# clawrim/gcn10

Hardware: AMD Instinct MI355X
Metric: CN Gpixels/sec (higher is better)
Workload: dtype u8

## Files before the change

gcn10_amd/csrc/gcn10_deflate_fused.hip:

```cpp
#include <hip/hip_runtime.h>

#include <cstdint>
#include <cstring>

#include "gcn10_deflate_internal.hpp"
#include "gcn10_gpu.h"
#include "gcn10_gpu_internal.hpp"

using gcn10::as_stream;
using gcn10::fail;
using gcn10::u32x4;
using gcn10::use_device;
using namespace gcn10_deflate;

namespace {

constexpr int kGroup = 6;

struct FusedJob {
    const uint8_t *esa;
    const uint8_t *hx;
    const int32_t *cj;
    const uint8_t *class_of;
    uint16_t *tok;
// ... 1338 lines not shown
    if (!ctx->d_hx || ctx->hx_W == 0 || (uint32_t)W != ctx->hx_W)
        return fail(GCN10_E_STATE, "gcn10_gpu_deflate_fused_strip: call gcn10_gpu_prepare_tile for W=%d first", W);
    if (W <= 0 || rows < 0 || cond_mask == 0 || (cond_mask & ~3u) || table_mask == 0 ||
        (table_mask >> ctx->n_tables))
        return fail(GCN10_E_INVAL, "gcn10_gpu_deflate_fused_strip: bad shape or masks");
    if (rows == 0)
        return GCN10_OK;
    if (!esa || !cj || !arena_dev || !table_dev || !cursor_dev)
        return fail(GCN10_E_INVAL, "gcn10_gpu_deflate_fused_strip: null pointer");
    if ((reinterpret_cast<uintptr_t>(arena_dev) & 15u) != 0)
        return fail(GCN10_E_INVAL, "gcn10_gpu_deflate_fused_strip: arena must be 16-byte aligned");

    FusedJob job;
    memset(&job, 0, sizeof job);
    job.esa = esa;
    job.hx = ctx->d_hx;
    job.cj = cj;
    job.class_of = ctx->d_class_of;
    job.hx_stride = ctx->hx_stride;
    job.hx_rows = ctx->hx_rows;
    job.seg_align = (uint32_t)ctx->arena_segment_align;
    for (int r = 0; r < GCN10_N_RASTERS; r++)
        if ((cond_mask >> (r / 9)) & 1u && (table_mask >> (r % 9)) & 1u)
            job.sel[job.n_sel++] = (uint8_t)r;
    job.t.arena = arena_dev;
    job.t.table = table_dev;
    job.t.cursor = cursor_dev;
    job.t.W = (uint32_t)W;
    job.t.rows = (uint32_t)rows;
    job.t.across = ((uint32_t)W + kTile - 1) / kTile;
    job.t.down = ((uint32_t)rows + kTile - 1) / kTile;
// ... 62 lines not shown
```

gcn10_amd/csrc/gcn10_gpu.hip:

```cpp

#include <hip/hip_runtime.h>
#include <unistd.h>
#include <hip/hip_ext.h>

#include <cstdarg>
#include <cstdint>
#include <cstdio>
#include <cstdlib>
#include <cstring>
#include <new>

#include "gcn10_gpu.h"
#include "gcn10_gpu_internal.hpp"

using gcn10::as_stream;
using gcn10::fail;
using gcn10::u32x4;
using gcn10::use_device;

namespace {

constexpr int kThreads = 256;
constexpr int kPxPerLane = 16;
constexpr int kChunk = kThreads * kPxPerLane;
// ... 11 lines not shown
    const uint8_t *hx;
    const int32_t *cj;
    const uint8_t *lut;
    uint8_t *out[GCN10_N_RASTERS];
    uint32_t W;
    uint32_t rows;
    uint32_t npix;
    uint32_t nvec16;
    uint32_t hx_stride;
    uint32_t hx_rows;
    uint32_t nchunks;
    uint32_t table_mask;
    uint32_t single_k;
    uint32_t xcd_slabs;
    const uint32_t *hx4;
    const uint32_t *hx4_complex;
    uint32_t hx4_stride;
    uint32_t hx4_gen;
};

__host__ __device__ inline uint8_t soil_code(uint8_t h)
{
    uint8_t d, u;
    if (h >= 11 && h <= 14) {
        d = 4;
        u = (uint8_t)(h - 10);
    }
    else {
        d = u = (h < 5) ? h : (uint8_t)kInvalidPlane;
    }
    return (uint8_t)(d | (u << 4));
}

// ... 80 lines not shown
        uint32_t lo = xcd * per;
        uint32_t hi = lo + per < nchunks ? lo + per : nchunks;
        step = nb / 8u;
        end = hi;
        return lo + (b >> 3);
    }
    step = nb;
    end = nchunks;
    return b;
}

enum { kLut16 = 0, kLut1 = 1 };
constexpr uint32_t kWavePx = 64u * kPxPerLane;
constexpr uint32_t kMinVectorW = kWavePx + 16u;

template <int ILP>
struct Trip {
    u32x4 e16[ILP], c16[ILP];
    uint32_t i0[ILP];
};

template <int ILP, bool NT, bool HX4>
__device__ __forceinline__ void issue_trip(const StripParams &p, uint32_t trip, uint32_t lane_off,
                                           uint32_t wave_off, Trip<ILP> &tr)
{
    uint32_t xb[ILP], r0[ILP], r1[ILP], wb[ILP];
#pragma unroll
    for (int u = 0; u < ILP; u++) {
        wb[u] = __builtin_amdgcn_readfirstlane((trip * ILP + u) * (uint32_t)kChunk + wave_off);
        const uint32_t wbc = wb[u] < p.npix ? wb[u] : 0u;
        const uint32_t y = wbc / p.W;
        xb[u] = wbc - y * p.W;
        r0[u] = (uint32_t)scalar_load_i32(p.cj, y);
        r1[u] = (uint32_t)scalar_load_i32(p.cj, y + 1u < p.rows ? y + 1u : y);
    }
#pragma unroll
    for (int u = 0; u < ILP; u++) {
        tr.i0[u] = wb[u] + lane_off;
        const uint8_t *pe = p.esa + (tr.i0[u] < p.nvec16 ? tr.i0[u] : 0u);
        tr.e16[u] = NT ? load16_aligned_nt(pe) : load16_aligned(pe);
    }
#pragma unroll
    for (int u = 0; u < ILP; u++) {
        uint32_t xl = xb[u] + lane_off;
        const bool wrap = xl >= p.W;
        xl = wrap ? xl - p.W : xl;
        const uint32_t row = clamp_row(p, (int32_t)(wrap ? r1[u] : r0[u]));
        if (HX4) {
            tr.c16[u] = u32x4{ p.hx4[(size_t)row * p.hx4_stride + (xl >> 4)], 0u, 0u, 0u };
            continue;
        }
        const uint8_t *pa = p.hx + (size_t)row * p.hx_stride + xl;
        u32x4 a = load16_any(pa);
        if (p.W & 15u) {
            const uint32_t n = p.W - xl;
            const bool strad = !wrap && n < (uint32_t)kPxPerLane;
            if (__builtin_amdgcn_ballot_w64(strad) != 0ull) {
                const uint8_t *pb = strad ? p.hx + (size_t)clamp_row(p, (int32_t)r1[u]) * p.hx_stride - n : pa;
                const u32x4 b = load16_any(pb);
                const uint32_t nn = strad ? n : (uint32_t)kPxPerLane;
#pragma unroll
                for (int j = 0; j < 4; j++) {
                    const int32_t m = (int32_t)nn - 4 * j;
                    const uint32_t mask = m >= 4 ? 0xffffffffu : (m <= 0 ? 0u : (1u << (8 * m)) - 1u);
// ... 7 lines not shown

__device__ __forceinline__ u32x4 expand_soil_word(uint32_t w)
{
    const uint32_t a = (w & 0xffu) * 0x01010101u, b = ((w >> 8) & 0xffu) * 0x01010101u;
    const int32_t split = (int32_t)((w >> 16) & 0xffu);
    u32x4 cd;
#pragma unroll
    for (int j = 0; j < 4; j++) {
        const int32_t m = split - 4 * j;
        const uint32_t mask = m >= 4 ? 0xffffffffu : (m <= 0 ? 0u : (1u << (8 * m)) - 1u);
        cd[j] = (a & mask) | (b & ~mask);
    }
    return cd;
}

template <int KIND, int COND_MASK, int ILP, bool NT, bool HX4>
__device__ __forceinline__ void finish_trip(const StripParams &p, const uint8_t *lut, uint32_t tmask,
                                            const Trip<ILP> &tr)
{
#pragma unroll
    for (int u = 0; u < ILP; u++) {
        const bool live = tr.i0[u] < p.nvec16;
        const u32x4 c16 = HX4 ? expand_soil_word(tr.c16[u][0]) : tr.c16[u];
#pragma unroll
        for (int c = 0; c < 2; c++) {
            if (!(COND_MASK & (1 << c)))
                continue;
            if (KIND == kLut16) {
                uint32_t acc[9][4];
#pragma unroll
                for (int j = 0; j < 4; j++) {
                    const uint32_t e = tr.e16[u][j];
                    const uint32_t cd = c16[j];
                    u32x4 r4[4];
#pragma unroll
                    for (int q = 0; q < 4; q++) {
                        const uint32_t lc16 = q == 0 ? (e << 4) & 0xff0u : (e >> (8 * q - 4)) & 0xff0u;
                        const uint32_t s = (cd >> (8 * q + 4 * c)) & 0xfu;
// ... 27 lines not shown
                    for (int q = 0; q < 4; q++) {
                        const uint32_t lc = (e >> (8 * q)) & 0xffu;
                        const uint32_t s = (cd >> (8 * q + 4 * c)) & 0xfu;
                        const uint32_t b = lut[s * (uint32_t)kPlane1 + lc];
                        w |= b << (8 * q);
                    }
                    v[j] = w;
                }
                if (live)
                    store16<NT>(p.out[c * 9 + p.single_k] + tr.i0[u], v);
            }
        }
    }
}

template <int KIND, int COND_MASK, int ILP, bool NT, bool PF, bool HX4>
__device__ __forceinline__ void strip_loop(const StripParams &p, const uint8_t *lut, uint32_t tmask,
                                           uint32_t lane_off, uint32_t wave_off)
{
    uint32_t step, end;
    uint32_t trip = first_chunk(p.nchunks, step, end, p.xcd_slabs != 0);
    if (!PF) {
        for (; trip < end; trip += step) {
            Trip<ILP> tr;
            issue_trip<ILP, NT, HX4>(p, trip, lane_off, wave_off, tr);
            finish_trip<KIND, COND_MASK, ILP, NT, HX4>(p, lut, tmask, tr);
        }
    }
    else if (trip < end) {
        Trip<ILP> ta, tb;
        issue_trip<ILP, NT, HX4>(p, trip, lane_off, wave_off, ta);
        for (;;) {
            trip += step;
            if (trip >= end) {
                finish_trip<KIND, COND_MASK, ILP, NT, HX4>(p, lut, tmask, ta);
                break;
            }
            issue_trip<ILP, NT, HX4>(p, trip, lane_off, wave_off, tb);
            finish_trip<KIND, COND_MASK, ILP, NT, HX4>(p, lut, tmask, ta);
            trip += step;
            if (trip >= end) {
                finish_trip<KIND, COND_MASK, ILP, NT, HX4>(p, lut, tmask, tb);
                break;
            }
            issue_trip<ILP, NT, HX4>(p, trip, lane_off, wave_off, ta);
            finish_trip<KIND, COND_MASK, ILP, NT, HX4>(p, lut, tmask, tb);
        }
    }
}

template <int KIND, int COND_MASK, bool ALL_TABLES, int ILP, bool NT, bool PF>
__global__ __launch_bounds__(kThreads) void cn_strip_kernel(const StripParams p)
{
    constexpr int kLutBytes = KIND == kLut16 ? kLut16Bytes : kLut1Bytes;
    __shared__ __attribute__((aligned(16))) uint8_t lut[kLutBytes];

    if (KIND == kLut16) {
        const u32x4 *src = reinterpret_cast<const u32x4 *>(p.lut);
        u32x4 *dst = reinterpret_cast<u32x4 *>(lut);
        for (int i = threadIdx.x; i < kLutBytes / 16; i += kThreads)
            dst[i] = src[i];
    }
    else {
        const uint32_t *src = reinterpret_cast<const uint32_t *>(p.lut);
        uint32_t *dst = reinterpret_cast<uint32_t *>(lut);
        for (int i = threadIdx.x; i < kLutBytes / 4; i += kThreads)
            dst[i] = src[i];
    }
    __syncthreads();

    const uint32_t lane_off = (threadIdx.x & 63u) * kPxPerLane;
    const uint32_t wave_off = __builtin_amdgcn_readfirstlane(threadIdx.x >> 6) * kWavePx;
    const uint32_t tmask = ALL_TABLES ? 0x1ffu : p.table_mask;

    if (p.hx4 && (uint32_t)scalar_load_i32(reinterpret_cast<const int32_t *>(p.hx4_complex), 0u) != p.hx4_gen)
        strip_loop<KIND, COND_MASK, ILP, NT, PF, true>(p, lut, tmask, lane_off, wave_off);
    else
        strip_loop<KIND, COND_MASK, ILP, NT, PF, false>(p, lut, tmask, lane_off, wave_off);

    if (blockIdx.x == 0 && threadIdx.x < p.npix - p.nvec16) {
        const uint32_t i = p.nvec16 + threadIdx.x;
        const uint32_t y = i / p.W;
        const uint32_t x = i - y * p.W;
        const uint32_t lc = p.esa[i];
        const uint32_t cd = p.hx[(size_t)soil_row(p, y) * p.hx_stride + x];
#pragma unroll
        for (int c = 0; c < 2; c++) {
            if (!(COND_MASK & (1 << c)))
                continue;
            const uint32_t s = (cd >> (4 * c)) & 0xfu;
            if (KIND == kLut16) {
                const uint8_t *row = lut + s * (uint32_t)kPlane16 + lc * 16u;
                for (int k = 0; k < 9; k++)
// ... 40 lines not shown
        const uint32_t x = i - y * p.W;
        const uint32_t lc = p.esa[i];
        const uint32_t cd = p.hx[(size_t)soil_row(p, y) * p.hx_stride + x];
        for (int c = 0; c < 2; c++) {
            if (!(cond_mask & (1u << c)))
                continue;
            const uint32_t s = (cd >> (4 * c)) & 0xfu;
            const uint8_t *row = lut + s * (uint32_t)kPlane16 + lc * 16u;
            for (int k = 0; k < 9; k++)
                if (p.table_mask & (1u << k))
                    p.out[c * 9 + k][i] = row[k];
        }
    }
}

constexpr uint32_t kExpandRows = 4;

template <bool VEC>
__global__ __launch_bounds__(kThreads) void expand_x_codes(const uint8_t *coarse,
                                                           uint32_t hsx, uint32_t hsy,
                                                           const int32_t *ci, uint32_t W,
                                                           uint8_t *hx, uint32_t hx_stride,
                                                           uint32_t *hx4, uint32_t *complex, uint32_t gen)
{
    const uint32_t x = (blockIdx.x * blockDim.x + threadIdx.x) * 16u;
    const uint32_t r0 = blockIdx.y * kExpandRows;
    if (x >= hx_stride || r0 >= hsy)
        return;
    const uint8_t pad = (uint8_t)(kInvalidPlane | (kInvalidPlane << 4));
    uint32_t cx[16];
    if (VEC && x + 16u <= W) {
        const u32x4 *civ = reinterpret_cast<const u32x4 *>(ci + x);
#pragma unroll
        for (int j = 0; j < 4; j++) {
            const u32x4 c4 = civ[j];
#pragma unroll
            for (int q = 0; q < 4; q++)
                cx[4 * j + q] = c4[q] < hsx ? c4[q] : hsx - 1u;
        }
    }
    else {
#pragma unroll
        for (int q = 0; q < 16; q++) {
            const uint32_t xx = x + q;
            const uint32_t c = xx < W ? (uint32_t)ci[xx] : 0u;
            cx[q] = xx < W ? (c < hsx ? c : hsx - 1u) : 0xffffffffu;
        }
    }
    const uint32_t c_lo = cx[0], c_hi = cx[15];
    const uint32_t r1 = r0 + kExpandRows < hsy ? r0 + kExpandRows : hsy;
    uint32_t split = 0;
    bool compact = true, in_set = true;
#pragma unroll
    for (int q = 0; q < 16; q++) {
        const bool lo = cx[q] == c_lo;
        in_set = in_set && (lo || cx[q] == c_hi);
        compact = compact && (lo ? split == (uint32_t)q : cx[q] == c_hi);
        split += lo && split == (uint32_t)q ? 1u : 0u;
    }
    const bool two = c_lo != 0xffffffffu && c_hi != 0xffffffffu && in_set;
    if (hx4 && x < W && !compact && *reinterpret_cast<volatile uint32_t *>(complex) != gen)
        *reinterpret_cast<volatile uint32_t *>(complex) = gen;
    for (uint32_t r = r0; r < r1; r++) {
        const uint8_t *row = coarse + (size_t)r * hsx;
        u32x4 o;
        if (two) {
            const uint32_t code_lo = soil_code(row[c_lo]), code_hi = soil_code(row[c_hi]);
#pragma unroll
            for (int j = 0; j < 4; j++) {
                uint32_t w = 0;
#pragma unroll
                for (int q = 0; q < 4; q++)
                    w |= (cx[4 * j + q] == c_lo ? code_lo : code_hi) << (8 * q);
                o[j] = w;
            }
        }
        else {
#pragma unroll
            for (int j = 0; j < 4; j++) {
                uint32_t w = 0;
#pragma unroll
                for (int q = 0; q < 4; q++) {
                    const uint32_t c = cx[4 * j + q];
                    const uint8_t code = c == 0xffffffffu ? pad : soil_code(row[c]);
                    w |= (uint32_t)code << (8 * q);
                }
                o[j] = w;
            }
        }
        __builtin_nontemporal_store(o, reinterpret_cast<u32x4 *>(hx + (size_t)r * hx_stride + x));
        if (hx4)
            __builtin_nontemporal_store(compact ? (o[0] & 0xffu) | ((o[3] >> 24) << 8) | (split << 16) : 0x00ff0000u,
                                        hx4 + (size_t)r * (hx_stride / 16u) + x / 16u);
    }
}

__global__ __launch_bounds__(kThreads) void resample_rows(const uint8_t *coarse,
                                                          uint32_t hsx,
                                                          const int32_t *ci,
                                                          const int32_t *cj, uint32_t W,
                                                          uint32_t rows, uint8_t *out)
{
    const size_t npix = (size_t)W * rows;
    const size_t stride = (size_t)gridDim.x * blockDim.x;
    for (size_t i = (size_t)blockIdx.x * blockDim.x + threadIdx.x; i < npix; i += stride) {
        const uint32_t y = (uint32_t)(i / W);
        const uint32_t x = (uint32_t)(i - (size_t)y * W);
        out[i] = coarse[(size_t)(uint32_t)cj[y] * hsx + (uint32_t)ci[x]];
// ... 183 lines not shown
{
    return s ? reinterpret_cast<hipStream_t>(s) : ctx->main_stream;
}

int grow_workspace(void **ws, size_t *cap, size_t need)
{
    if (need <= *cap)
        return GCN10_OK;
    HIP_TRY(hipDeviceSynchronize());
    if (*ws)
        HIP_TRY(hipFree(*ws));
    *ws = nullptr;
    *cap = 0;
    HIP_TRY(hipMalloc(ws, need));
    *cap = need;
    return GCN10_OK;
}

}

namespace {

uint32_t stream_grid(const gcn10_gpu_ctx *ctx, uint64_t nchunks, int blocks_per_cu = 0)
{
    uint64_t cap = (uint64_t)ctx->n_cus * (blocks_per_cu > 0 ? blocks_per_cu : ctx->grid_blocks_per_cu);
    cap -= cap % 8u;
    if (cap < 8)
        cap = 8;
    uint64_t g = nchunks < cap ? nchunks : cap;
    return (uint32_t)(g ? g : 1);
// ... 38 lines not shown
    HIP_TRY(hipGetDeviceProperties(&prop, device));
    if (strncmp(prop.gcnArchName, "gfx950", 6) != 0)
        return fail(GCN10_E_NODEVICE, "device %d is %s; this library carries gfx950 code only",
                    device, prop.gcnArchName);

    gcn10_gpu_ctx *ctx = new (std::nothrow) gcn10_gpu_ctx();
    if (!ctx)
        return fail(GCN10_E_NOMEM, "context allocation failed");
    ctx->device = device;
    ctx->n_cus = prop.multiProcessorCount;
    hipError_t e2 = hipStreamCreateWithFlags(&ctx->main_stream, hipStreamNonBlocking);
    if (e2 == hipSuccess)
        e2 = hipMalloc(reinterpret_cast<void **>(&ctx->d_lut16), kLut16Bytes);
    if (e2 == hipSuccess)
        e2 = hipMalloc(reinterpret_cast<void **>(&ctx->d_lut1), GCN10_N_TABLES * kLut1Bytes);
    if (e2 != hipSuccess) {
        int rc = fail(GCN10_E_HIP, "context setup: %s", hipGetErrorString(e2));
        gcn10_gpu_destroy(ctx);
        return rc;
    }
    *out = ctx;
    return GCN10_OK;
}

void gcn10_gpu_destroy(gcn10_gpu_ctx *ctx)
{
    if (!ctx)
        return;
    (void)hipSetDevice(ctx->device);
    if (ctx->main_stream) {
        (void)hipStreamSynchronize(ctx->main_stream);
        (void)hipStreamDestroy(ctx->main_stream);
    }
    if (ctx->d_lut16)
        (void)hipFree(ctx->d_lut16);
    if (ctx->d_lut1)
        (void)hipFree(ctx->d_lut1);
    if (ctx->d_hx_alloc)
        (void)hipFree(ctx->d_hx_alloc);
    if (ctx->deflate_ws)
        (void)hipFree(ctx->deflate_ws);
    if (ctx->inflate_ws)
        (void)hipFree(ctx->inflate_ws);
    if (ctx->lzw_ws)
        (void)hipFree(ctx->lzw_ws);
    if (ctx->d_class_of)
        (void)hipFree(ctx->d_class_of);
    delete ctx;
}

int gcn10_gpu_device_info(gcn10_gpu_ctx *ctx, char *name, size_t cap, size_t *hbm_bytes)
{
    int rc = use_device(ctx);
    if (rc)
// ... 369 lines not shown
    return GCN10_OK;
}


int gcn10_gpu_prepare_tile(gcn10_gpu_ctx *ctx, const uint8_t *coarse, int hsx, int hsy,
                           const int32_t *ci, int W, gcn10_stream_t stream)
{
    int rc = use_device(ctx);
    if (rc)
        return rc;
    if (hsx <= 0 || hsy <= 0 || W <= 0)
        return fail(GCN10_E_INVAL, "gcn10_gpu_prepare_tile: bad shape W=%d soil=%dx%d", W, hsx, hsy);
    if (!coarse || !ci)
        return fail(GCN10_E_INVAL, "gcn10_gpu_prepare_tile: null pointer");
    const uint32_t stride = (((uint32_t)W + 15u) & ~15u) + 16u;
    const size_t need = (size_t)stride * (size_t)hsy;
    if (need > ctx->hx_capacity) {
        HIP_TRY(hipDeviceSynchronize());
        if (ctx->d_hx_alloc)
            HIP_TRY(hipFree(ctx->d_hx_alloc));
        ctx->d_hx_alloc = ctx->d_hx = nullptr;
        ctx->d_hx4 = ctx->d_hx4_complex = nullptr;
        ctx->hx4_ready = false;
        ctx->hx_capacity = 0;
        const size_t need16 = (need + 15) & ~(size_t)15;
        HIP_TRY(hipMalloc(reinterpret_cast<void **>(&ctx->d_hx_alloc), 16 + need16 + need16 / 4 + 16));
        ctx->d_hx = ctx->d_hx_alloc + 16;
        ctx->d_hx4 = reinterpret_cast<uint32_t *>(ctx->d_hx + need16);
        ctx->d_hx4_complex = reinterpret_cast<uint32_t *>(ctx->d_hx + need16 + need16 / 4);
        HIP_TRY(hipMemsetAsync(ctx->d_hx4_complex, 0, 4, as_stream(ctx, stream)));
        ctx->hx4_gen = 0;
        ctx->hx_capacity = need;
    }
    uint32_t *hx4 = ctx->compact_soil ? ctx->d_hx4 : nullptr;
    ctx->hx4_ready = hx4 != nullptr;
    if (hx4 && ++ctx->hx4_gen == 0u)
        ctx->hx4_gen = 1u;
    ctx->hx_stride = stride;
    ctx->hx_W = (uint32_t)W;
    ctx->hx_rows = (uint32_t)hsy;
    dim3 grid((stride / 16 + kThreads - 1) / kThreads, ((uint32_t)hsy + kExpandRows - 1) / kExpandRows);
    if (aligned16(ci))
        hipLaunchKernelGGL(expand_x_codes<true>, grid, dim3(kThreads), 0, as_stream(ctx, stream),
                           coarse, (uint32_t)hsx, (uint32_t)hsy, ci, (uint32_t)W, ctx->d_hx, stride, hx4,
                           ctx->d_hx4_complex, ctx->hx4_gen);
    else
        hipLaunchKernelGGL(expand_x_codes<false>, grid, dim3(kThreads), 0, as_stream(ctx, stream),
                           coarse, (uint32_t)hsx, (uint32_t)hsy, ci, (uint32_t)W, ctx->d_hx, stride, hx4,
                           ctx->d_hx4_complex, ctx->hx4_gen);
    HIP_TRY(hipGetLastError());
    return GCN10_OK;
}

int gcn10_gpu_cn_strip(gcn10_gpu_ctx *ctx, const uint8_t *esa, int W, int rows,
                       const int32_t *cj, unsigned cond_mask, unsigned table_mask,
                       uint8_t *const out[GCN10_N_RASTERS], gcn10_stream_t stream)
{
    int rc = use_device(ctx);
    if (rc)
        return rc;
    if (ctx->n_tables == 0)
        return fail(GCN10_E_STATE, "gcn10_gpu_cn_strip: call gcn10_gpu_set_tables first");
    if (!ctx->d_hx || ctx->hx_W == 0)
        return fail(GCN10_E_STATE, "gcn10_gpu_cn_strip: call gcn10_gpu_prepare_tile first");
    if (W <= 0 || rows < 0 || (uint32_t)W != ctx->hx_W)
// ... 14 lines not shown
    StripParams p;
    memset(&p, 0, sizeof p);
    bool all_aligned = aligned16(esa);
    for (int c = 0; c < 2; c++) {
        for (int k = 0; k < 9; k++) {
            const int r = c * 9 + k;
            if ((cond_mask & (1u << c)) && (table_mask & (1u << k))) {
                if (!out[r])
                    return fail(GCN10_E_INVAL, "gcn10_gpu_cn_strip: out[%d] is null but selected", r);
                p.out[r] = out[r];
                all_aligned = all_aligned && aligned16(out[r]);
            }
        }
    }
    p.esa = esa;
    p.hx = ctx->d_hx;
    p.cj = cj;
    p.W = (uint32_t)W;
    p.rows = (uint32_t)rows;
    p.npix = (uint32_t)((uint64_t)W * (uint64_t)rows);
    p.hx_stride = ctx->hx_stride;
    p.hx_rows = ctx->hx_rows;
    p.nchunks = (p.npix + kChunk - 1) / kChunk;
    p.table_mask = table_mask;
    hipStream_t s = as_stream(ctx, stream);

    p.xcd_slabs = (uint32_t)ctx->xcd_slabs;
    p.nvec16 = p.npix & ~15u;
    if (ctx->hx4_ready && ctx->compact_soil && (p.W & 15u) == 0u) {
        p.hx4 = ctx->d_hx4;
        p.hx4_complex = ctx->d_hx4_complex;
        p.hx4_stride = ctx->hx_stride / 16u;
        p.hx4_gen = ctx->hx4_gen;
    }
    if (p.npix < 16u || p.W < kMinVectorW)
        all_aligned = false;
    if (!all_aligned) {
        p.lut = ctx->d_lut16;
        const uint32_t g = stream_grid(ctx, ((uint64_t)p.npix + kThreads - 1) / kThreads);
        if (ctx->time_start && ctx->time_stop) {
            void *args[] = { &p, &cond_mask };
            HIP_TRY(hipExtLaunchKernel(reinterpret_cast<const void *>(cn_strip_bytes), dim3(g), dim3(kThreads), args, 0,
                                       s, ctx->time_start, ctx->time_stop, 0));
            ctx->time_start = ctx->time_stop = nullptr;
        }
        else {
            hipLaunchKernelGGL(cn_strip_bytes, dim3(g), dim3(kThreads), 0, s, p, cond_mask);
        }
        ctx->last_kernel = "cn_strip_bytes";
    }
    else {
// ... 225 lines not shown
        *best_ms = best;
    if (report && report_cap)
        snprintf(report, report_cap,
                 "{\"positions\": %d, \"step_bytes\": %zu, \"shapes\": %zu, \"best_ms\": %.4f, \"worst_ms\": %.4f, "
                 "\"best_offset_bytes\": %zu, \"xcd_slabs\": %d, \"grid_blocks_per_cu\": %d, \"ilp1\": %d, \"prefetch\": %d}",
                 n_pos, step, sizeof shapes / sizeof shapes[0], best, worst, best_pos, best_shape.xcd, best_shape.bpc,
                 best_shape.ilp, best_shape.pf);
    return GCN10_OK;
}

int gcn10_gpu_soil_words_state(gcn10_gpu_ctx *ctx, gcn10_stream_t stream)
{
    int rc = use_device(ctx);
    if (rc)
        return rc;
    if (!ctx->hx4_ready || !ctx->d_hx4_complex)
        return 0;
    uint32_t flag = 0;
    hipStream_t s = as_stream(ctx, stream);
    HIP_TRY(hipMemcpyAsync(&flag, ctx->d_hx4_complex, 4, hipMemcpyDeviceToHost, s));
    HIP_TRY(hipStreamSynchronize(s));
    return flag == ctx->hx4_gen ? 2 : 1;
}

const char *gcn10_gpu_last_kernel_name(gcn10_gpu_ctx *ctx)
{
    return ctx ? ctx->last_kernel : "";
}

}
```

gcn10_amd/csrc/gcn10_gpu_internal.hpp:

```cpp
#ifndef GCN10_GPU_INTERNAL_HPP
#define GCN10_GPU_INTERNAL_HPP

#include <hip/hip_runtime.h>

#include <cstdint>

#include "gcn10_gpu.h"

namespace gcn10 {

int fail(int code, const char *fmt, ...) __attribute__((format(printf, 2, 3)));

#define HIP_TRY(expr)                                                                   \
    do {                                                                                \
        hipError_t e_ = (expr);                                                         \
        if (e_ != hipSuccess)                                                           \
            return gcn10::fail(e_ == hipErrorOutOfMemory ? GCN10_E_NOMEM : GCN10_E_HIP, \
                               "%s: %s", #expr, hipGetErrorString(e_));                 \
    } while (0)

int use_device(gcn10_gpu_ctx *ctx);
hipStream_t as_stream(gcn10_gpu_ctx *ctx, gcn10_stream_t s);
int grow_workspace(void **ws, size_t *cap, size_t need);

typedef uint32_t u32x4 __attribute__((ext_vector_type(4)));

__device__ __forceinline__ bool inflate_window_ok(uint32_t out_len, uint32_t chunk_w, uint32_t src_x, uint32_t src_y,
                                                  uint32_t copy_w, uint32_t copy_h, uint32_t slot_bytes)
{
    if (copy_w == 0 || copy_h == 0)
        return true;
    if (chunk_w == 0 || out_len > slot_bytes || src_x > chunk_w || copy_w > chunk_w - src_x)
        return false;
    const unsigned long long last = (unsigned long long)(src_y + copy_h - 1u) * chunk_w + src_x + copy_w;
    return (unsigned long long)src_y + copy_h <= 0xffffffffull && last <= out_len;
}

void launch_lzw_decode(const uint8_t *comp_dev, const gcn10_inflate_tile *tiles_dev, uint32_t n_tiles,
// ... 4 lines not shown
constexpr int kLut16Plane = 256 * 16 + 16;
constexpr int kLut16Bytes = 6 * kLut16Plane;

}

struct gcn10_gpu_ctx {
    int device = -1;
    int n_cus = 0;
    hipStream_t main_stream = nullptr;
    uint8_t *d_lut16 = nullptr;
    uint8_t *d_lut1 = nullptr;
    int n_tables = 0;
    uint8_t *d_hx = nullptr;
    uint8_t *d_hx_alloc = nullptr;
    uint32_t *d_hx4 = nullptr;
    uint32_t *d_hx4_complex = nullptr;
    uint32_t hx4_gen = 0;
    bool hx4_ready = false;
    int compact_soil = 1;
    size_t hx_capacity = 0;
    uint32_t hx_stride = 0;
    uint32_t hx_W = 0;
    uint32_t hx_rows = 0;
    const char *last_kernel = "";
    char kernel_name[96] = "";
    int grid_blocks_per_cu = 16;
    int ilp16 = 0;
    int ilp1 = 2;
    int nontemporal = 1;
    int xcd_slabs = 1;
    int prefetch = 1;
    struct SingleShape {
        bool set = false;
        int xcd_slabs = 1, grid_blocks_per_cu = 8, ilp = 2, prefetch = 1;
// ... 22 lines not shown
```

gcn10_amd/csrc/gcn10_overview.hip:

```cpp
#include <hip/hip_runtime.h>

#include <cstdint>

#include "gcn10_gpu_internal.hpp"

using namespace gcn10;

namespace {

constexpr int kThreads = 256;
constexpr int kPlanes = 6;
constexpr int kPlane16 = 256 * 16 + 16;
constexpr int kLut16Bytes = kPlanes * kPlane16;
constexpr int kMaxLevels = 8;
constexpr int kL1Tile = 128;
constexpr uint32_t kL1Rows = 4;

__device__ __forceinline__ uint8_t avg_of(uint32_t s, uint32_t n)
{
    return n == 0 ? (uint8_t)GCN10_NODATA : (uint8_t)((2u * s + n) / (2u * n));
}

struct NearestParams {
    const uint8_t *src;
// ... 173 lines not shown
        return rc;
    if (ctx->n_tables == 0)
        return fail(GCN10_E_STATE, "gcn10_gpu_overview_average: call gcn10_gpu_set_tables first");
    if (!ctx->d_hx || (int)ctx->hx_W != W)
        return fail(GCN10_E_STATE, "gcn10_gpu_overview_average: prepare the block's tile (W=%d) first", W);
    if (!esa || !cj || !levels || W <= 0 || H <= 0 || n_levels < 1 || n_levels > kMaxLevels || y0 < 0 ||
        rows <= 0 || y0 % 256 != 0 || y0 + rows > H || (rows % 256 != 0 && y0 + rows != H))
        return fail(GCN10_E_INVAL, "gcn10_gpu_overview_average: bad strip y0=%d rows=%d of %dx%d, %d levels "
                    "(strips start and end on multiples of 256 rows, 1..8 levels)", y0, rows, W, H, n_levels);
    if (cond_mask == 0 || (cond_mask & ~3u) || table_mask == 0 || (table_mask >> ctx->n_tables) != 0)
        return fail(GCN10_E_INVAL, "gcn10_gpu_overview_average: bad masks cond=%#x table=%#x", cond_mask, table_mask);
    AvgParams p = {};
    p.esa = esa;
    p.cj = cj;
    p.lut16 = ctx->d_lut16;
    p.hx = ctx->d_hx;
    p.hx_stride = ctx->hx_stride;
    p.hx_rows = ctx->hx_rows;
    p.W = (uint32_t)W;
    p.H = (uint32_t)H;
    p.cond_mask = cond_mask;
    p.table_mask = table_mask;
    p.n_levels = (uint32_t)n_levels;
    int q = 0;
    for (int r = 0; r < GCN10_N_RASTERS; r++) {
        if (!((cond_mask >> (r / 9)) & 1u) || !((table_mask >> (r % 9)) & 1u))
            continue;
        for (int k = 0; k < n_levels; k++) {
            p.out[r][k] = levels[q * n_levels + k];
            if (!p.out[r][k])
                return fail(GCN10_E_INVAL, "gcn10_gpu_overview_average: level %d of raster %d is NULL", k + 1, r);
// ... 21 lines not shown
```

gcn10_amd/csrc/gcn10_stats.hip:

```cpp
#include <hip/hip_runtime.h>

#include <cstdint>

#include "gcn10_gpu_internal.hpp"
#include "gcn10_pair_hist.hpp"

using namespace gcn10;
using namespace gcn10::pair_hist;

namespace {

constexpr uint32_t kChunk = kThreads * kPxPerLane;
constexpr uint32_t kRowsPerItem = 4;
constexpr int kGridPerCu = 4;

struct HistParams {
    const uint8_t *esa;
    const uint8_t *hx;
    const int32_t *cj;
    unsigned long long *hist;
    uint32_t W, rows, hx_stride, hx_rows, per_row;
};

__global__ __launch_bounds__(kThreads) void pair_histogram_kernel(const HistParams p)
// ... 63 lines not shown

int gcn10_gpu_pair_histogram(gcn10_gpu_ctx *ctx, const uint8_t *esa, int W, int rows, const int32_t *cj,
                             unsigned long long *hist_dev, gcn10_stream_t stream)
{
    int rc = use_device(ctx);
    if (rc)
        return rc;
    if (!ctx->d_hx || (int)ctx->hx_W != W)
        return fail(GCN10_E_STATE, "gcn10_gpu_pair_histogram: prepare the block's tile (W=%d) first", W);
    if (!esa || !cj || !hist_dev || W <= 0 || rows < 0)
        return fail(GCN10_E_INVAL, "gcn10_gpu_pair_histogram: bad arguments W=%d rows=%d", W, rows);
    if (rows == 0)
        return GCN10_OK;
    HistParams p = {};
    p.esa = esa;
    p.hx = ctx->d_hx;
    p.cj = cj;
    p.hist = hist_dev;
    p.W = (uint32_t)W;
    p.rows = (uint32_t)rows;
    p.hx_stride = ctx->hx_stride;
    p.hx_rows = ctx->hx_rows;
    p.per_row = ((uint32_t)W + kChunk - 1u) / kChunk;
    const uint64_t items = (uint64_t)((p.rows + kRowsPerItem - 1u) / kRowsPerItem) * p.per_row;
    const uint64_t cap = (uint64_t)(ctx->n_cus > 0 ? ctx->n_cus : 256) * kGridPerCu;
    const uint32_t grid = (uint32_t)(items < cap ? items : cap);
    hipLaunchKernelGGL(pair_histogram_kernel, dim3(grid), dim3(kThreads), 0, as_stream(ctx, stream), p);
    HIP_TRY(hipGetLastError());
    return GCN10_OK;
}

// ... 2 lines not shown
```

gcn10_amd/csrc/gcn10_verify.hip:

```cpp
#include <hip/hip_runtime.h>

#include <cstdint>
#include <cstring>

#include "gcn10_gpu_internal.hpp"

using namespace gcn10;

namespace {

constexpr int kThreads = 256;
constexpr uint32_t kPxPerLane = 16;
constexpr int kGridPerCu = 4;

struct VerifyParams {
    const uint8_t *esa;
    const uint8_t *hx;
    const int32_t *cj;
    const uint8_t *lut;
    const uint8_t *want[GCN10_N_RASTERS];
    const uint8_t *got[GCN10_N_RASTERS];
    gcn10_verify_count *counts;
    uint64_t want_stride, got_stride;
    uint32_t W, rows, y0;
// ... 318 lines not shown
        return GCN10_OK;
    if (!esa || !cj || !got || !counts_dev)
        return fail(GCN10_E_INVAL, "gcn10_gpu_verify_strip: null pointer");
    for (int c = 0; c < GCN10_N_CONDS; c++) {
        for (int k = 0; k < GCN10_N_TABLES; k++) {
            const int r = c * GCN10_N_TABLES + k;
            if (!(cond_mask & (1u << c)) || !(table_mask & (1u << k)))
                continue;
            if (!got[r])
                return fail(GCN10_E_INVAL, "gcn10_gpu_verify_strip: got[%d] is null but selected", r);
            p.got[r] = got[r];
            p.sel |= 1u << r;
        }
    }
    p.esa = esa;
    p.hx = ctx->d_hx;
    p.cj = cj;
    p.lut = ctx->d_lut16;
    p.counts = counts_dev;
    p.hx_stride = ctx->hx_stride;
    p.hx_rows = ctx->hx_rows;
    hipStream_t s = as_stream(ctx, stream);
    if (p.sel == (1u << GCN10_N_RASTERS) - 1u)
        hipLaunchKernelGGL(verify_strip_kernel<true>, dim3(grid_for(ctx, p)), dim3(kThreads), 0, s, p);
    else
        hipLaunchKernelGGL(verify_strip_kernel<false>, dim3(grid_for(ctx, p)), dim3(kThreads), 0, s, p);
    HIP_TRY(hipGetLastError());
    hipLaunchKernelGGL(verify_first_kernel<true>, dim3(1), dim3(64), 0, s, p);
    HIP_TRY(hipGetLastError());
    return GCN10_OK;
}
// ... 42 lines not shown
```

gcn10_amd/csrc/gcn10_zonal.hip:

```cpp
#include <hip/hip_runtime.h>

#include <cstdint>

#include "gcn10_gpu_internal.hpp"
#include "gcn10_pair_hist.hpp"

using namespace gcn10;
using namespace gcn10::pair_hist;

namespace {

constexpr int kZonalGridPerCu = 4;
constexpr uint32_t kWaves = kThreads / 64;

struct ZonalParams {
    const uint8_t *esa;
    const uint8_t *hx;
    const int32_t *cj;
    const gcn10_zone_span *spans;
    const gcn10_zone_item *items;
    unsigned long long *hist;
    uint32_t W, hx_stride, hx_rows, n_items, items_per_wg;
};

// ... 124 lines not shown
                                   int n_zones, unsigned long long *hist_dev, gcn10_stream_t stream)
{
    int rc = use_device(ctx);
    if (rc)
        return rc;
    if (n_items == 0)
        return GCN10_OK;
    if (!ctx->d_hx || (int)ctx->hx_W != W)
        return fail(GCN10_E_STATE, "gcn10_gpu_zonal_pair_histogram: prepare the block's tile (W=%d) first", W);
    if (!esa || !cj || !spans_dev || !items_dev || !hist_dev || W <= 0 || rows <= 0 || n_zones <= 0 ||
        n_items > 0xffffffffu)
        return fail(GCN10_E_INVAL, "gcn10_gpu_zonal_pair_histogram: bad arguments W=%d rows=%d zones=%d items=%zu", W,
                    rows, n_zones, n_items);
    ZonalParams p = {};
    p.esa = esa;
    p.hx = ctx->d_hx;
    p.cj = cj;
    p.spans = spans_dev;
    p.items = items_dev;
    p.hist = hist_dev;
    p.W = (uint32_t)W;
    p.hx_stride = ctx->hx_stride;
    p.hx_rows = ctx->hx_rows;
    p.n_items = (uint32_t)n_items;
    const uint64_t cap = (uint64_t)(ctx->n_cus > 0 ? ctx->n_cus : 256) * kZonalGridPerCu;
    const uint32_t grid = (uint32_t)(n_items < cap ? n_items : cap);
    p.items_per_wg = (p.n_items + grid - 1u) / grid;
    hipLaunchKernelGGL(zonal_pair_histogram_kernel, dim3(grid), dim3(kThreads), 0, as_stream(ctx, stream), p);
    HIP_TRY(hipGetLastError());
    return GCN10_OK;
}
// ... 3 lines not shown
```

Baseline: 2889.

## Build compact soil tables in prepare_tile and expand byte plane lazily

prepare_tile now runs a single kernel that writes per-row soil code bytes, clamped column indices, and the compact 16-pixel soil words, instead of always expanding the full byte-per-pixel hx plane. The full hx plane is built on demand by soil_bytes, which records an event, only for consumers that need it. The CN strip kernel gains a third path that gathers codes per pixel through cx when tiles are not compact, so the hx plane can be skipped there too. This avoids writing the large expanded plane when only the compact path is used, at the cost of an extra lazy kernel and per-pixel gathers in the complex case.

```diff
diff --git a/gcn10_amd/csrc/gcn10_deflate_fused.hip b/gcn10_amd/csrc/gcn10_deflate_fused.hip
--- a/gcn10_amd/csrc/gcn10_deflate_fused.hip
+++ b/gcn10_amd/csrc/gcn10_deflate_fused.hip
@@ -1376,7 +1376,8 @@
     FusedJob job;
     memset(&job, 0, sizeof job);
     job.esa = esa;
-    job.hx = ctx->d_hx;
+    if ((rc = gcn10::soil_bytes(ctx, gcn10::as_stream(ctx, stream), &job.hx)) != GCN10_OK)
+        return rc;
     job.cj = cj;
     job.class_of = ctx->d_class_of;
     job.hx_stride = ctx->hx_stride;
diff --git a/gcn10_amd/csrc/gcn10_gpu.hip b/gcn10_amd/csrc/gcn10_gpu.hip
--- a/gcn10_amd/csrc/gcn10_gpu.hip
+++ b/gcn10_amd/csrc/gcn10_gpu.hip
@@ -49,9 +49,12 @@
     uint32_t single_k;
     uint32_t xcd_slabs;
     const uint32_t *hx4;
-    const uint32_t *hx4_complex;
     uint32_t hx4_stride;
-    uint32_t hx4_gen;
+    const uint32_t *cx;
+    const uint8_t *codes;
+    uint32_t codes_stride;
+    const uint32_t *soil_complex;
+    uint32_t soil_gen;
 };
 
 __host__ __device__ inline uint8_t soil_code(uint8_t h)
@@ -162,13 +165,15 @@
 constexpr uint32_t kWavePx = 64u * kPxPerLane;
 constexpr uint32_t kMinVectorW = kWavePx + 16u;
 
+enum { kSoilBytes = 0, kSoilWords = 1, kSoilPixels = 2 };
+
 template <int ILP>
 struct Trip {
     u32x4 e16[ILP], c16[ILP];
     uint32_t i0[ILP];
 };
 
-template <int ILP, bool NT, bool HX4>
+template <int ILP, bool NT, int SOIL>
 __device__ __forceinline__ void issue_trip(const StripParams &p, uint32_t trip, uint32_t lane_off,
                                            uint32_t wave_off, Trip<ILP> &tr)
 {
@@ -194,8 +199,25 @@
         const bool wrap = xl >= p.W;
         xl = wrap ? xl - p.W : xl;
         const uint32_t row = clamp_row(p, (int32_t)(wrap ? r1[u] : r0[u]));
-        if (HX4) {
+        if (SOIL == kSoilWords) {
             tr.c16[u] = u32x4{ p.hx4[(size_t)row * p.hx4_stride + (xl >> 4)], 0u, 0u, 0u };
+            continue;
+        }
+        if (SOIL == kSoilPixels) {
+            const uint8_t *cr = p.codes + (size_t)row * p.codes_stride;
+            const u32x4 *pc = reinterpret_cast<const u32x4 *>(p.cx + xl);
+            u32x4 a = { 0u, 0u, 0u, 0u };
+#pragma unroll 1
+            for (int j = 0; j < 4; j++) {
+                const u32x4 c4 = pc[j];
+                const uint32_t w = (uint32_t)cr[c4[0]] | (uint32_t)cr[c4[1]] << 8 | (uint32_t)cr[c4[2]] << 16 |
+                                   (uint32_t)cr[c4[3]] << 24;
+                a[0] = j == 0 ? w : a[0];
+                a[1] = j == 1 ? w : a[1];
+                a[2] = j == 2 ? w : a[2];
+                a[3] = j == 3 ? w : a[3];
+            }
+            tr.c16[u] = a;
             continue;
         }
         const uint8_t *pa = p.hx + (size_t)row * p.hx_stride + xl;
@@ -233,14 +255,14 @@
     return cd;
 }
 
-template <int KIND, int COND_MASK, int ILP, bool NT, bool HX4>
+template <int KIND, int COND_MASK, int ILP, bool NT, int SOIL>
 __device__ __forceinline__ void finish_trip(const StripParams &p, const uint8_t *lut, uint32_t tmask,
                                             const Trip<ILP> &tr)
 {
 #pragma unroll
     for (int u = 0; u < ILP; u++) {
         const bool live = tr.i0[u] < p.nvec16;
-        const u32x4 c16 = HX4 ? expand_soil_word(tr.c16[u][0]) : tr.c16[u];
+        const u32x4 c16 = SOIL == kSoilWords ? expand_soil_word(tr.c16[u][0]) : tr.c16[u];
 #pragma unroll
         for (int c = 0; c < 2; c++) {
             if (!(COND_MASK & (1 << c)))
@@ -298,37 +320,39 @@
     }
 }
 
-template <int KIND, int COND_MASK, int ILP, bool NT, bool PF, bool HX4>
+template <int KIND, int COND_MASK, int ILP, bool NT, bool PF, int SOIL>
 __device__ __forceinline__ void strip_loop(const StripParams &p, const uint8_t *lut, uint32_t tmask,
                                            uint32_t lane_off, uint32_t wave_off)
 {
     uint32_t step, end;
     uint32_t trip = first_chunk(p.nchunks, step, end, p.xcd_slabs != 0);
+    if (trip >= end)
+        return;
     if (!PF) {
         for (; trip < end; trip += step) {
             Trip<ILP> tr;
-            issue_trip<ILP, NT, HX4>(p, trip, lane_off, wave_off, tr);
-            finish_trip<KIND, COND_MASK, ILP, NT, HX4>(p, lut, tmask, tr);
-        }
-    }
-    else if (trip < end) {
+            issue_trip<ILP, NT, SOIL>(p, trip, lane_off, wave_off, tr);
+            finish_trip<KIND, COND_MASK, ILP, NT, SOIL>(p, lut, tmask, tr);
+        }
+    }
+    else {
         Trip<ILP> ta, tb;
-        issue_trip<ILP, NT, HX4>(p, trip, lane_off, wave_off, ta);
+        issue_trip<ILP, NT, SOIL>(p, trip, lane_off, wave_off, ta);
         for (;;) {
             trip += step;
             if (trip >= end) {
-                finish_trip<KIND, COND_MASK, ILP, NT, HX4>(p, lut, tmask, ta);
+                finish_trip<KIND, COND_MASK, ILP, NT, SOIL>(p, lut, tmask, ta);
                 break;
             }
-            issue_trip<ILP, NT, HX4>(p, trip, lane_off, wave_off, tb);
-            finish_trip<KIND, COND_MASK, ILP, NT, HX4>(p, lut, tmask, ta);
+            issue_trip<ILP, NT, SOIL>(p, trip, lane_off, wave_off, tb);
+            finish_trip<KIND, COND_MASK, ILP, NT, SOIL>(p, lut, tmask, ta);
             trip += step;
             if (trip >= end) {
-                finish_trip<KIND, COND_MASK, ILP, NT, HX4>(p, lut, tmask, tb);
+                finish_trip<KIND, COND_MASK, ILP, NT, SOIL>(p, lut, tmask, tb);
                 break;
             }
-            issue_trip<ILP, NT, HX4>(p, trip, lane_off, wave_off, ta);
-            finish_trip<KIND, COND_MASK, ILP, NT, HX4>(p, lut, tmask, tb);
+            issue_trip<ILP, NT, SOIL>(p, trip, lane_off, wave_off, ta);
+            finish_trip<KIND, COND_MASK, ILP, NT, SOIL>(p, lut, tmask, tb);
         }
     }
 }
@@ -357,10 +381,12 @@
     const uint32_t wave_off = __builtin_amdgcn_readfirstlane(threadIdx.x >> 6) * kWavePx;
     const uint32_t tmask = ALL_TABLES ? 0x1ffu : p.table_mask;
 
-    if (p.hx4 && (uint32_t)scalar_load_i32(reinterpret_cast<const int32_t *>(p.hx4_complex), 0u) != p.hx4_gen)
-        strip_loop<KIND, COND_MASK, ILP, NT, PF, true>(p, lut, tmask, lane_off, wave_off);
+    if (!p.hx4)
+        strip_loop<KIND, COND_MASK, ILP, NT, PF, kSoilBytes>(p, lut, tmask, lane_off, wave_off);
+    else if ((uint32_t)scalar_load_i32(reinterpret_cast<const int32_t *>(p.soil_complex), 0u) != p.soil_gen)
+        strip_loop<KIND, COND_MASK, ILP, NT, PF, kSoilWords>(p, lut, tmask, lane_off, wave_off);
     else
-        strip_loop<KIND, COND_MASK, ILP, NT, PF, false>(p, lut, tmask, lane_off, wave_off);
+        strip_loop<KIND, COND_MASK, ILP, NT, PF, kSoilPixels>(p, lut, tmask, lane_off, wave_off);
 
     if (blockIdx.x == 0 && threadIdx.x < p.npix - p.nvec16) {
         const uint32_t i = p.nvec16 + threadIdx.x;
@@ -431,58 +457,126 @@
     }
 }
 
+constexpr uint32_t kWordRows = 8;
+
+template <bool VEC>
+__global__ __launch_bounds__(kThreads) void soil_tables_kernel(const uint8_t *coarse, uint32_t hsx, uint32_t hsy,
+                                                               const int32_t *ci, uint32_t W, uint32_t hx_stride,
+                                                               uint32_t word_chunks, uint8_t *codes,
+                                                               uint32_t codes_stride, uint32_t *cx_out, uint32_t *hx4,
+                                                               uint32_t *complex, uint32_t gen)
+{
+    const uint32_t pad = (uint32_t)(kInvalidPlane | (kInvalidPlane << 4));
+    if (blockIdx.y >= word_chunks) {
+        const uint32_t per_row = codes_stride / 16u;
+        const uint32_t t = ((blockIdx.y - word_chunks) * gridDim.x + blockIdx.x) * blockDim.x + threadIdx.x;
+        const uint32_t r = t / per_row;
+        if (r >= hsy)
+            return;
+        const uint32_t c0 = (t - r * per_row) * 16u;
+        const uint8_t *row = coarse + (size_t)r * hsx;
+        u32x4 in = { 0u, 0u, 0u, 0u };
+        if (c0 + 16u <= hsx) {
+            in = load16_any(row + c0);
+        }
+        else {
+#pragma unroll
+            for (int q = 0; q < 16; q++)
+                if (c0 + q < hsx)
+                    in[q >> 2] |= (uint32_t)row[c0 + q] << (8 * (q & 3));
+        }
+        u32x4 o;
+#pragma unroll
+        for (int j = 0; j < 4; j++) {
+            uint32_t w = 0;
+#pragma unroll
+            for (int q = 0; q < 4; q++) {
+                const uint32_t code = c0 + 4 * j + q < hsx ? soil_code((uint8_t)(in[j] >> (8 * q))) : pad;
+                w |= code << (8 * q);
+            }
+            o[j] = w;
+        }
+        *reinterpret_cast<u32x4 *>(codes + (size_t)r * codes_stride + c0) = o;
+        return;
+    }
+    const uint32_t x = (blockIdx.x * blockDim.x + threadIdx.x) * 16u;
+    const uint32_t r0 = blockIdx.y * kWordRows;
+    if (x >= hx_stride || r0 >= hsy)
+        return;
+    uint32_t cx[16];
+    if (VEC && x + 16u <= W) {
+        const u32x4 *civ = reinterpret_cast<const u32x4 *>(ci + x);
+#pragma unroll
+        for (int j = 0; j < 4; j++) {
+            const u32x4 c4 = civ[j];
+#pragma unroll
+            for (int q = 0; q < 4; q++)
+                cx[4 * j + q] = c4[q] < hsx ? c4[q] : hsx - 1u;
+        }
+    }
+    else {
+#pragma unroll
+        for (int q = 0; q < 16; q++) {
+            const uint32_t xx = x + q;
+            const uint32_t c = xx < W ? (uint32_t)ci[xx] : 0u;
+            cx[q] = xx < W ? (c < hsx ? c : hsx - 1u) : hsx;
+        }
+    }
+    const uint32_t c_lo = cx[0], c_hi = cx[15];
+    uint32_t split = 0;
+    bool compact = true;
+#pragma unroll
+    for (int q = 0; q < 16; q++) {
+        const bool lo = cx[q] == c_lo;
+        compact = compact && (lo ? split == (uint32_t)q : cx[q] == c_hi);
+        split += lo && split == (uint32_t)q ? 1u : 0u;
+    }
+    if (blockIdx.y == 0) {
+#pragma unroll
+        for (int j = 0; j < 4; j++)
+            *reinterpret_cast<u32x4 *>(cx_out + x + 4 * j) =
+                u32x4{ cx[4 * j], cx[4 * j + 1], cx[4 * j + 2], cx[4 * j + 3] };
+        if (x < W && !compact && *reinterpret_cast<volatile uint32_t *>(complex) != gen)
+            *reinterpret_cast<volatile uint32_t *>(complex) = gen;
+    }
+    const uint32_t r1 = r0 + kWordRows < hsy ? r0 + kWordRows : hsy;
+    for (uint32_t r = r0; r < r1; r++) {
+        const uint8_t *row = coarse + (size_t)r * hsx;
+        const uint32_t a = c_lo < hsx ? soil_code(row[c_lo]) : pad, b = c_hi < hsx ? soil_code(row[c_hi]) : pad;
+        __builtin_nontemporal_store(compact ? a | (b << 8) | (split << 16) : 0x00ff0000u,
+                                    hx4 + (size_t)r * (hx_stride / 16u) + x / 16u);
+    }
+}
+
 constexpr uint32_t kExpandRows = 4;
 
-template <bool VEC>
-__global__ __launch_bounds__(kThreads) void expand_x_codes(const uint8_t *coarse,
-                                                           uint32_t hsx, uint32_t hsy,
-                                                           const int32_t *ci, uint32_t W,
-                                                           uint8_t *hx, uint32_t hx_stride,
-                                                           uint32_t *hx4, uint32_t *complex, uint32_t gen)
+__global__ __launch_bounds__(kThreads) void expand_code_bytes(const uint8_t *codes, uint32_t codes_stride,
+                                                              uint32_t hsy, const uint32_t *cx_in, uint8_t *hx,
+                                                              uint32_t hx_stride)
 {
     const uint32_t x = (blockIdx.x * blockDim.x + threadIdx.x) * 16u;
     const uint32_t r0 = blockIdx.y * kExpandRows;
     if (x >= hx_stride || r0 >= hsy)
         return;
-    const uint8_t pad = (uint8_t)(kInvalidPlane | (kInvalidPlane << 4));
     uint32_t cx[16];
-    if (VEC && x + 16u <= W) {
-        const u32x4 *civ = reinterpret_cast<const u32x4 *>(ci + x);
-#pragma unroll
-        for (int j = 0; j < 4; j++) {
-            const u32x4 c4 = civ[j];
-#pragma unroll
-            for (int q = 0; q < 4; q++)
-                cx[4 * j + q] = c4[q] < hsx ? c4[q] : hsx - 1u;
-        }
-    }
-    else {
-#pragma unroll
-        for (int q = 0; q < 16; q++) {
-            const uint32_t xx = x + q;
-            const uint32_t c = xx < W ? (uint32_t)ci[xx] : 0u;
-            cx[q] = xx < W ? (c < hsx ? c : hsx - 1u) : 0xffffffffu;
-        }
+#pragma unroll
+    for (int j = 0; j < 4; j++) {
+        const u32x4 c4 = *reinterpret_cast<const u32x4 *>(cx_in + x + 4 * j);
+#pragma unroll
+        for (int q = 0; q < 4; q++)
+            cx[4 * j + q] = c4[q];
     }
     const uint32_t c_lo = cx[0], c_hi = cx[15];
+    bool two = true;
+#pragma unroll
+    for (int q = 0; q < 16; q++)
+        two = two && (cx[q] == c_lo || cx[q] == c_hi);
     const uint32_t r1 = r0 + kExpandRows < hsy ? r0 + kExpandRows : hsy;
-    uint32_t split = 0;
-    bool compact = true, in_set = true;
-#pragma unroll
-    for (int q = 0; q < 16; q++) {
-        const bool lo = cx[q] == c_lo;
-        in_set = in_set && (lo || cx[q] == c_hi);
-        compact = compact && (lo ? split == (uint32_t)q : cx[q] == c_hi);
-        split += lo && split == (uint32_t)q ? 1u : 0u;
-    }
-    const bool two = c_lo != 0xffffffffu && c_hi != 0xffffffffu && in_set;
-    if (hx4 && x < W && !compact && *reinterpret_cast<volatile uint32_t *>(complex) != gen)
-        *reinterpret_cast<volatile uint32_t *>(complex) = gen;
     for (uint32_t r = r0; r < r1; r++) {
-        const uint8_t *row = coarse + (size_t)r * hsx;
+        const uint8_t *row = codes + (size_t)r * codes_stride;
         u32x4 o;
         if (two) {
-            const uint32_t code_lo = soil_code(row[c_lo]), code_hi = soil_code(row[c_hi]);
+            const uint32_t code_lo = row[c_lo], code_hi = row[c_hi];
 #pragma unroll
             for (int j = 0; j < 4; j++) {
                 uint32_t w = 0;
@@ -497,18 +591,12 @@
             for (int j = 0; j < 4; j++) {
                 uint32_t w = 0;
 #pragma unroll
-                for (int q = 0; q < 4; q++) {
-                    const uint32_t c = cx[4 * j + q];
-                    const uint8_t code = c == 0xffffffffu ? pad : soil_code(row[c]);
-                    w |= (uint32_t)code << (8 * q);
-                }
+                for (int q = 0; q < 4; q++)
+                    w |= (uint32_t)row[cx[4 * j + q]] << (8 * q);
                 o[j] = w;
             }
         }
         __builtin_nontemporal_store(o, reinterpret_cast<u32x4 *>(hx + (size_t)r * hx_stride + x));
-        if (hx4)
-            __builtin_nontemporal_store(compact ? (o[0] & 0xffu) | ((o[3] >> 24) << 8) | (split << 16) : 0x00ff0000u,
-                                        hx4 + (size_t)r * (hx_stride / 16u) + x / 16u);
     }
 }
 
@@ -722,6 +810,26 @@
     *cap = 0;
     HIP_TRY(hipMalloc(ws, need));
     *cap = need;
+    return GCN10_OK;
+}
+
+int soil_bytes(gcn10_gpu_ctx *ctx, hipStream_t stream, const uint8_t **hx)
+{
+    *hx = nullptr;
+    if (!ctx->d_hx || ctx->hx_W == 0)
+        return fail(GCN10_E_STATE, "no prepared tile: call gcn10_gpu_prepare_tile first");
+    if (!ctx->hx_made) {
+        dim3 grid((ctx->hx_stride / 16 + kThreads - 1) / kThreads, (ctx->hx_rows + kExpandRows - 1) / kExpandRows);
+        hipLaunchKernelGGL(expand_code_bytes, grid, dim3(kThreads), 0, stream, ctx->d_codes, ctx->codes_stride,
+                           ctx->hx_rows, ctx->d_cx, ctx->d_hx, ctx->hx_stride);
+        HIP_TRY(hipGetLastError());
+        HIP_TRY(hipEventRecord(ctx->hx_made_ev, stream));
+        ctx->hx_made = true;
+    }
+    else {
+        HIP_TRY(hipStreamWaitEvent(stream, ctx->hx_made_ev, 0));
+    }
+    *hx = ctx->d_hx;
     return GCN10_OK;
 }
 
@@ -790,6 +898,12 @@
         e2 = hipMalloc(reinterpret_cast<void **>(&ctx->d_lut16), kLut16Bytes);
     if (e2 == hipSuccess)
         e2 = hipMalloc(reinterpret_cast<void **>(&ctx->d_lut1), GCN10_N_TABLES * kLut1Bytes);
+    if (e2 == hipSuccess)
+        e2 = hipMalloc(reinterpret_cast<void **>(&ctx->d_soil_complex), 16);
+    if (e2 == hipSuccess)
+        e2 = hipMemset(ctx->d_soil_complex, 0, 16);
+    if (e2 == hipSuccess)
+        e2 = hipEventCreateWithFlags(&ctx->hx_made_ev, hipEventDisableTiming);
     if (e2 != hipSuccess) {
         int rc = fail(GCN10_E_HIP, "context setup: %s", hipGetErrorString(e2));
         gcn10_gpu_destroy(ctx);
@@ -814,6 +928,10 @@
         (void)hipFree(ctx->d_lut1);
     if (ctx->d_hx_alloc)
         (void)hipFree(ctx->d_hx_alloc);
+    if (ctx->d_soil_complex)
+        (void)hipFree(ctx->d_soil_complex);
+    if (ctx->hx_made_ev)
+        (void)hipEventDestroy(ctx->hx_made_ev);
     if (ctx->deflate_ws)
         (void)hipFree(ctx->deflate_ws);
     if (ctx->inflate_ws)
@@ -1213,41 +1331,47 @@
     if (!coarse || !ci)
         return fail(GCN10_E_INVAL, "gcn10_gpu_prepare_tile: null pointer");
     const uint32_t stride = (((uint32_t)W + 15u) & ~15u) + 16u;
-    const size_t need = (size_t)stride * (size_t)hsy;
+    const size_t need_hx = ((size_t)stride * (size_t)hsy + 63) & ~(size_t)63;
+    const uint32_t codes_stride = (((uint32_t)hsx + 1u) + 15u) & ~15u;
+    const size_t off_words = need_hx;
+    const size_t off_cx = (off_words + (size_t)(stride / 16u) * 4u * (size_t)hsy + 15) & ~(size_t)15;
+    const size_t off_codes = (off_cx + (size_t)stride * 4u + 15) & ~(size_t)15;
+    const size_t need = off_codes + (size_t)codes_stride * (size_t)hsy;
     if (need > ctx->hx_capacity) {
         HIP_TRY(hipDeviceSynchronize());
         if (ctx->d_hx_alloc)
             HIP_TRY(hipFree(ctx->d_hx_alloc));
         ctx->d_hx_alloc = ctx->d_hx = nullptr;
-        ctx->d_hx4 = ctx->d_hx4_complex = nullptr;
-        ctx->hx4_ready = false;
         ctx->hx_capacity = 0;
-        const size_t need16 = (need + 15) & ~(size_t)15;
-        HIP_TRY(hipMalloc(reinterpret_cast<void **>(&ctx->d_hx_alloc), 16 + need16 + need16 / 4 + 16));
+        ctx->hx_W = 0;
+        HIP_TRY(hipMalloc(reinterpret_cast<void **>(&ctx->d_hx_alloc), 16 + need));
         ctx->d_hx = ctx->d_hx_alloc + 16;
-        ctx->d_hx4 = reinterpret_cast<uint32_t *>(ctx->d_hx + need16);
-        ctx->d_hx4_complex = reinterpret_cast<uint32_t *>(ctx->d_hx + need16 + need16 / 4);
-        HIP_TRY(hipMemsetAsync(ctx->d_hx4_complex, 0, 4, as_stream(ctx, stream)));
-        ctx->hx4_gen = 0;
         ctx->hx_capacity = need;
     }
-    uint32_t *hx4 = ctx->compact_soil ? ctx->d_hx4 : nullptr;
-    ctx->hx4_ready = hx4 != nullptr;
-    if (hx4 && ++ctx->hx4_gen == 0u)
-        ctx->hx4_gen = 1u;
+    ctx->d_hx4 = reinterpret_cast<uint32_t *>(ctx->d_hx + off_words);
+    ctx->d_cx = reinterpret_cast<uint32_t *>(ctx->d_hx + off_cx);
+    ctx->d_codes = ctx->d_hx + off_codes;
+    ctx->codes_stride = codes_stride;
+    if (++ctx->soil_gen == 0u)
+        ctx->soil_gen = 1u;
+    ctx->hx_made = false;
     ctx->hx_stride = stride;
     ctx->hx_W = (uint32_t)W;
     ctx->hx_rows = (uint32_t)hsy;
-    dim3 grid((stride / 16 + kThreads - 1) / kThreads, ((uint32_t)hsy + kExpandRows - 1) / kExpandRows);
-    if (aligned16(ci))
-        hipLaunchKernelGGL(expand_x_codes<true>, grid, dim3(kThreads), 0, as_stream(ctx, stream),
-                           coarse, (uint32_t)hsx, (uint32_t)hsy, ci, (uint32_t)W, ctx->d_hx, stride, hx4,
-                           ctx->d_hx4_complex, ctx->hx4_gen);
-    else
-        hipLaunchKernelGGL(expand_x_codes<false>, grid, dim3(kThreads), 0, as_stream(ctx, stream),
-                           coarse, (uint32_t)hsx, (uint32_t)hsy, ci, (uint32_t)W, ctx->d_hx, stride, hx4,
-                           ctx->d_hx4_complex, ctx->hx4_gen);
+    hipStream_t s = as_stream(ctx, stream);
+    const uint32_t group_blocks = (stride / 16u + kThreads - 1) / kThreads;
+    const uint32_t word_chunks = ((uint32_t)hsy + kWordRows - 1) / kWordRows;
+    const size_t code_threads = (size_t)(codes_stride / 16u) * (size_t)hsy;
+    const uint32_t code_chunks = (uint32_t)((code_threads + (size_t)group_blocks * kThreads - 1) / ((size_t)group_blocks * kThreads));
+    auto fn = aligned16(ci) ? soil_tables_kernel<true> : soil_tables_kernel<false>;
+    hipLaunchKernelGGL(fn, dim3(group_blocks, word_chunks + code_chunks), dim3(kThreads), 0, s, coarse, (uint32_t)hsx,
+                       (uint32_t)hsy, ci, (uint32_t)W, stride, word_chunks, ctx->d_codes, codes_stride, ctx->d_cx,
+                       ctx->d_hx4, ctx->d_soil_complex, ctx->soil_gen);
     HIP_TRY(hipGetLastError());
+    if (!ctx->compact_soil || (W & 15)) {
+        const uint8_t *hx;
+        return gcn10::soil_bytes(ctx, s, &hx);
+    }
     return GCN10_OK;
 }
 
@@ -1292,7 +1416,6 @@
         }
     }
     p.esa = esa;
-    p.hx = ctx->d_hx;
     p.cj = cj;
     p.W = (uint32_t)W;
     p.rows = (uint32_t)rows;
@@ -1305,14 +1428,22 @@
 
     p.xcd_slabs = (uint32_t)ctx->xcd_slabs;
     p.nvec16 = p.npix & ~15u;
-    if (ctx->hx4_ready && ctx->compact_soil && (p.W & 15u) == 0u) {
-        p.hx4 = ctx->d_hx4;
-        p.hx4_complex = ctx->d_hx4_complex;
-        p.hx4_stride = ctx->hx_stride / 16u;
-        p.hx4_gen = ctx->hx4_gen;
-    }
     if (p.npix < 16u || p.W < kMinVectorW)
         all_aligned = false;
+    if (all_aligned && ctx->compact_soil && (p.W & 15u) == 0u) {
+        p.hx4 = ctx->d_hx4;
+        p.hx4_stride = ctx->hx_stride / 16u;
+        p.cx = ctx->d_cx;
+        p.codes = ctx->d_codes;
+        p.codes_stride = ctx->codes_stride;
+        p.soil_complex = ctx->d_soil_complex;
+        p.soil_gen = ctx->soil_gen;
+    }
+    else {
+        rc = gcn10::soil_bytes(ctx, s, &p.hx);
+        if (rc)
+            return rc;
+    }
     if (!all_aligned) {
         p.lut = ctx->d_lut16;
         const uint32_t g = stream_grid(ctx, ((uint64_t)p.npix + kThreads - 1) / kThreads);
@@ -1568,13 +1699,13 @@
     int rc = use_device(ctx);
     if (rc)
         return rc;
-    if (!ctx->hx4_ready || !ctx->d_hx4_complex)
+    if (!ctx->compact_soil || !ctx->d_hx || ctx->hx_W == 0)
         return 0;
     uint32_t flag = 0;
     hipStream_t s = as_stream(ctx, stream);
-    HIP_TRY(hipMemcpyAsync(&flag, ctx->d_hx4_complex, 4, hipMemcpyDeviceToHost, s));
+    HIP_TRY(hipMemcpyAsync(&flag, ctx->d_soil_complex, 4, hipMemcpyDeviceToHost, s));
     HIP_TRY(hipStreamSynchronize(s));
-    return flag == ctx->hx4_gen ? 2 : 1;
+    return flag == ctx->soil_gen ? 2 : 1;
 }
 
 const char *gcn10_gpu_last_kernel_name(gcn10_gpu_ctx *ctx)
diff --git a/gcn10_amd/csrc/gcn10_gpu_internal.hpp b/gcn10_amd/csrc/gcn10_gpu_internal.hpp
--- a/gcn10_amd/csrc/gcn10_gpu_internal.hpp
+++ b/gcn10_amd/csrc/gcn10_gpu_internal.hpp
@@ -22,6 +22,7 @@
 int use_device(gcn10_gpu_ctx *ctx);
 hipStream_t as_stream(gcn10_gpu_ctx *ctx, gcn10_stream_t s);
 int grow_workspace(void **ws, size_t *cap, size_t need);
+int soil_bytes(gcn10_gpu_ctx *ctx, hipStream_t stream, const uint8_t **hx);
 
 typedef uint32_t u32x4 __attribute__((ext_vector_type(4)));
 
@@ -56,10 +57,14 @@
     uint8_t *d_hx = nullptr;
     uint8_t *d_hx_alloc = nullptr;
     uint32_t *d_hx4 = nullptr;
-    uint32_t *d_hx4_complex = nullptr;
-    uint32_t hx4_gen = 0;
-    bool hx4_ready = false;
+    uint32_t *d_cx = nullptr;
+    uint8_t *d_codes = nullptr;
+    uint32_t codes_stride = 0;
+    uint32_t *d_soil_complex = nullptr;
+    uint32_t soil_gen = 0;
     int compact_soil = 1;
+    bool hx_made = false;
+    hipEvent_t hx_made_ev = nullptr;
     size_t hx_capacity = 0;
     uint32_t hx_stride = 0;
     uint32_t hx_W = 0;
diff --git a/gcn10_amd/csrc/gcn10_overview.hip b/gcn10_amd/csrc/gcn10_overview.hip
--- a/gcn10_amd/csrc/gcn10_overview.hip
+++ b/gcn10_amd/csrc/gcn10_overview.hip
@@ -211,7 +211,8 @@
     p.esa = esa;
     p.cj = cj;
     p.lut16 = ctx->d_lut16;
-    p.hx = ctx->d_hx;
+    if ((rc = gcn10::soil_bytes(ctx, gcn10::as_stream(ctx, stream), &p.hx)) != GCN10_OK)
+        return rc;
     p.hx_stride = ctx->hx_stride;
     p.hx_rows = ctx->hx_rows;
     p.W = (uint32_t)W;
diff --git a/gcn10_amd/csrc/gcn10_stats.hip b/gcn10_amd/csrc/gcn10_stats.hip
--- a/gcn10_amd/csrc/gcn10_stats.hip
+++ b/gcn10_amd/csrc/gcn10_stats.hip
@@ -101,7 +101,8 @@
         return GCN10_OK;
     HistParams p = {};
     p.esa = esa;
-    p.hx = ctx->d_hx;
+    if ((rc = gcn10::soil_bytes(ctx, gcn10::as_stream(ctx, stream), &p.hx)) != GCN10_OK)
+        return rc;
     p.cj = cj;
     p.hist = hist_dev;
     p.W = (uint32_t)W;
diff --git a/gcn10_amd/csrc/gcn10_verify.hip b/gcn10_amd/csrc/gcn10_verify.hip
--- a/gcn10_amd/csrc/gcn10_verify.hip
+++ b/gcn10_amd/csrc/gcn10_verify.hip
@@ -356,7 +356,8 @@
         }
     }
     p.esa = esa;
-    p.hx = ctx->d_hx;
+    if ((rc = gcn10::soil_bytes(ctx, gcn10::as_stream(ctx, stream), &p.hx)) != GCN10_OK)
+        return rc;
     p.cj = cj;
     p.lut = ctx->d_lut16;
     p.counts = counts_dev;
diff --git a/gcn10_amd/csrc/gcn10_zonal.hip b/gcn10_amd/csrc/gcn10_zonal.hip
--- a/gcn10_amd/csrc/gcn10_zonal.hip
+++ b/gcn10_amd/csrc/gcn10_zonal.hip
@@ -162,7 +162,8 @@
                     rows, n_zones, n_items);
     ZonalParams p = {};
     p.esa = esa;
-    p.hx = ctx->d_hx;
+    if ((rc = gcn10::soil_bytes(ctx, gcn10::as_stream(ctx, stream), &p.hx)) != GCN10_OK)
+        return rc;
     p.cj = cj;
     p.spans = spans_dev;
     p.items = items_dev;
```

Measured after the change: 2925 (median of 6 runs). 1.3% higher.
